# tencent-ailab/pika

Measured on NVIDIA H100. Metric: utterances/sec RNN-T train step (T=1000,U=150,V=6k), higher is better.
Workload: dtype bf16

## Files before the change

pika_b200/csrc/rnnt_loss.cu:

```cuda
#include <cstdlib>

#include "../../include/pika_b200.h"
#include "common.cuh"

namespace pk {
void count_launch();

constexpr float kLog2e = 1.4426950408889634f;
constexpr float kLn2 = 0.6931471805599453f;

template <typename T> struct Vec16;
template <> struct Vec16<__nv_bfloat16> {
    static constexpr int N = 8;
    PK_DEVICE static void unpack(const uint4& q, float (&f)[8]) {
        f[0] = bf16lo(q.x); f[1] = bf16hi(q.x); f[2] = bf16lo(q.y); f[3] = bf16hi(q.y);
        f[4] = bf16lo(q.z); f[5] = bf16hi(q.z); f[6] = bf16lo(q.w); f[7] = bf16hi(q.w);
    }
    PK_DEVICE static uint4 pack(const float (&f)[8]) {
        return make_uint4(pack_bf16x2(f[0], f[1]), pack_bf16x2(f[2], f[3]), pack_bf16x2(f[4], f[5]), pack_bf16x2(f[6], f[7]));
    }
    PK_DEVICE static float vmax(const uint4& q) {
        const __nv_bfloat162 a = __hmax2(*reinterpret_cast<const __nv_bfloat162*>(&q.x), *reinterpret_cast<const __nv_bfloat162*>(&q.y));
        const __nv_bfloat162 b = __hmax2(*reinterpret_cast<const __nv_bfloat162*>(&q.z), *reinterpret_cast<const __nv_bfloat162*>(&q.w));
        const __nv_bfloat162 c = __hmax2(a, b);
        return fmaxf(__low2float(c), __high2float(c));
    }
};
template <> struct Vec16<float> {
    static constexpr int N = 4;
    PK_DEVICE static void unpack(const uint4& q, float (&f)[4]) {
        f[0] = __uint_as_float(q.x); f[1] = __uint_as_float(q.y); f[2] = __uint_as_float(q.z); f[3] = __uint_as_float(q.w);
    }
    PK_DEVICE static uint4 pack(const float (&f)[4]) {
        return make_uint4(__float_as_uint(f[0]), __float_as_uint(f[1]), __float_as_uint(f[2]), __float_as_uint(f[3]));
    }
    PK_DEVICE static float vmax(const uint4& q) {
        return fmaxf(fmaxf(__uint_as_float(q.x), __uint_as_float(q.y)), fmaxf(__uint_as_float(q.z), __uint_as_float(q.w)));
    }
};

PK_DEVICE uint4 ld_stream(const uint4* p) {
    uint4 r;
    asm volatile("ld.global.nc.L1::no_allocate.v4.u32 {%0,%1,%2,%3}, [%4];" : "=r"(r.x), "=r"(r.y), "=r"(r.z), "=r"(r.w) : "l"(p));
    return r;
}
PK_DEVICE uint4 ld_plain(const uint4* p) { return *p; }
PK_DEVICE void st_stream(uint4* p, const uint4& v) {
    asm volatile("st.global.cs.v4.u32 [%0], {%1,%2,%3,%4};" ::"l"(p), "r"(v.x), "r"(v.y), "r"(v.z), "r"(v.w) : "memory");
}

struct RnntDims {
    int B, T, U1, V, ldv;
    int ld_labels;
    int ND;
};
PK_DEVICE size_t skew_index(const RnntDims& d, int b, int t, int u) { return ((size_t)b * d.ND + (t + u)) * d.U1 + u; }

constexpr int ROWSTATS_UNROLL = 4;

template <typename T>
__global__ void __launch_bounds__(256) rnnt_rowstats_kernel(const T* __restrict__ logits, const int* __restrict__ labels,
                                                            const int* __restrict__ frame_lens, const int* __restrict__ label_lens,
                                                            RnntDims d, float* __restrict__ lse_out, float* __restrict__ lpb_skew,
                                                            float* __restrict__ lpl_skew) {
    constexpr int VN = Vec16<T>::N;
    const int lane = threadIdx.x & 31;
    const long long warp_global = (long long)blockIdx.x * (blockDim.x >> 5) + (threadIdx.x >> 5);
    const long long n_warps = (long long)gridDim.x * (blockDim.x >> 5);
    const long long rows = (long long)d.B * d.T * d.U1;
    const int nvec = (d.V + VN - 1) / VN;
    for (long long row = warp_global; row < rows; row += n_warps) {
        const int u = (int)(row % d.U1);
        const long long bt = row / d.U1;
        const int t = (int)(bt % d.T);
        const int b = (int)(bt / d.T);
        const int Tn = frame_lens[b], Un = label_lens[b];
        if (t >= Tn || u > Un) continue;
        const T* rp = logits + row * (long long)d.ldv;
        const uint4* vp = reinterpret_cast<const uint4*>(rp);
        float m = -INFINITY, s = 0.f;
        const int nfull = d.V / VN;
        for (int i0 = lane; i0 < nfull; i0 += 32 * ROWSTATS_UNROLL) {
            uint4 q[ROWSTATS_UNROLL];
#pragma unroll
            for (int k = 0; k < ROWSTATS_UNROLL; ++k) {
                const int i = i0 + k * 32;
                if (i < nfull) q[k] = ld_stream(vp + i);
            }
#pragma unroll
            for (int k = 0; k < ROWSTATS_UNROLL; ++k) {
                const int i = i0 + k * 32;
                if (i < nfull) {
                    const float cm = Vec16<T>::vmax(q[k]) * kLog2e;
                    if (cm > m) { s *= exp2f(m - cm); m = cm; }
                    float f[VN];
                    Vec16<T>::unpack(q[k], f);
#pragma unroll
                    for (int e = 0; e < VN; ++e) s += ex2_approx(fmaf(f[e], kLog2e, -m));
                }
            }
        }
        if (nfull * VN < d.V && lane == 0) {
            for (int v = nfull * VN; v < d.V; ++v) {
                const float x = to_f32<T>(rp[v]) * kLog2e;
                if (x > m) { s *= exp2f(m - x); m = x; }
                s += exp2f(x - m);
            }
        }
        const float mw = warp_max(m);
        s = (m == -INFINITY) ? 0.f : s * exp2f(m - mw);
        s = warp_sum(s);
        if (lane == 0) {
            const float lse = (mw + log2f(s)) * kLn2;
            const float zb = to_f32<T>(rp[0]);
            lse_out[row] = lse;
            const size_t sk = skew_index(d, b, t, u);
            lpb_skew[sk] = zb - lse;
            if (u < Un) {
                const int y = labels[(size_t)b * d.ld_labels + u];
                lpl_skew[sk] = to_f32<T>(rp[y]) - lse;
            }
        }
    }
}

template <typename T>
__global__ void __launch_bounds__(256) rnnt_rowfinish_kernel(const T* __restrict__ logits, const int* __restrict__ labels,
                                                             const int* __restrict__ frame_lens, const int* __restrict__ label_lens,
                                                             RnntDims d, const float2* __restrict__ parts, int n_parts,
                                                             float* __restrict__ lse_out, float* __restrict__ lpb_skew,
                                                             float* __restrict__ lpl_skew) {
    const long long rows = (long long)d.B * d.T * d.U1;
    for (long long row = (long long)blockIdx.x * blockDim.x + threadIdx.x; row < rows; row += (long long)gridDim.x * blockDim.x) {
        const int u = (int)(row % d.U1);
        const long long bt = row / d.U1;
        const int t = (int)(bt % d.T);
        const int b = (int)(bt / d.T);
        const int Tn = frame_lens[b], Un = label_lens[b];
        if (t >= Tn || u > Un) continue;
        float m = -INFINITY;
        for (int i = 0; i < n_parts; ++i) m = fmaxf(m, parts[(size_t)i * rows + row].x);
        float sum = 0.f;
        for (int i = 0; i < n_parts; ++i) {
            const float2 ps = parts[(size_t)i * rows + row];
            sum += ps.y * exp2f(ps.x - m);
        }
        const float lse = (m + log2f(sum)) * kLn2;
        const T* rp = logits + row * (long long)d.ldv;
        lse_out[row] = lse;
        const size_t sk = skew_index(d, b, t, u);
        lpb_skew[sk] = to_f32<T>(rp[0]) - lse;
        if (u < Un) {
            const int y = labels[(size_t)b * d.ld_labels + u];
            lpl_skew[sk] = to_f32<T>(rp[y]) - lse;
        }
    }
}

typedef double lat_t;
#define LAT_NEG_INF (-(double)INFINITY)
PK_DEVICE lat_t lse2(lat_t a, lat_t b) {
    const lat_t mx = fmax(a, b), mn = fmin(a, b);
    if (mx == LAT_NEG_INF) return LAT_NEG_INF;
    return mx + log1p(exp(mn - mx));
}

constexpr int LAT_MAX_G = 512;
constexpr int LAT_MAX_CPT = 4;

__global__ void __launch_bounds__(2 * LAT_MAX_G) rnnt_lattice_kernel(
    const int* __restrict__ frame_lens, const int* __restrict__ label_lens, RnntDims d, int G, int cpt,
    const float* __restrict__ lpb_skew, const float* __restrict__ lpl_skew, lat_t* __restrict__ alpha_skew,
    lat_t* __restrict__ beta_skew, const float* __restrict__ grad_scale, float* __restrict__ costs,
    float* __restrict__ gb_out, float* __restrict__ gl_out) {
    extern __shared__ lat_t sm[];
    const int b = blockIdx.x;
    const int grp = threadIdx.x >= G ? 1 : 0;
    const int j = threadIdx.x - grp * G;
    const int T = frame_lens[b], U = label_lens[b];
    const int W = d.U1 + 2;
    lat_t* buf0 = sm + grp * 2 * W + 1;
    lat_t* buf1 = buf0 + W;
    __shared__ lat_t s_ll;
    const size_t base = (size_t)b * d.ND * d.U1;
    const bool valid = (T > 0 && T <= d.T && U >= 0 && U < d.U1);
    if (valid) {
        for (int i = j - 1; i <= d.U1; i += G) { buf0[i] = LAT_NEG_INF; buf1[i] = LAT_NEG_INF; }
        named_bar_sync(1 + grp, G);
        const int last = T - 1 + U;
        if (grp == 0) {
            lat_t* prev = buf0;
            lat_t* cur = buf1;
            if (j == 0) { cur[0] = 0.0; alpha_skew[base] = 0.0; }
            float nb[LAT_MAX_CPT], nl[LAT_MAX_CPT];
#pragma unroll
            for (int c = 0; c < LAT_MAX_CPT; ++c) {
                const int u = j + c * G;
                nb[c] = (c < cpt && u <= U && last >= 1) ? lpb_skew[base + u] : 0.f;
                nl[c] = (c < cpt && u >= 1 && u <= U && last >= 1) ? lpl_skew[base + u - 1] : 0.f;
            }
            named_bar_sync(1, G);
            for (int dg = 1; dg <= last; ++dg) {
                lat_t* tsw = prev; prev = cur; cur = tsw;
                const int lo = max(0, dg - (T - 1)), hi = min(U, dg);
                float pb[LAT_MAX_CPT], pl[LAT_MAX_CPT];
#pragma unroll
                for (int c = 0; c < LAT_MAX_CPT; ++c) { pb[c] = nb[c]; pl[c] = nl[c]; }
                if (dg < last) {
                    const size_t nbase = base + (size_t)dg * d.U1;
#pragma unroll
                    for (int c = 0; c < LAT_MAX_CPT; ++c) {
                        const int u = j + c * G;
                        if (c < cpt && u <= U) {
                            nb[c] = lpb_skew[nbase + u];
                            nl[c] = (u >= 1) ? lpl_skew[nbase + u - 1] : 0.f;
                        }
                    }
                }
#pragma unroll
                for (int c = 0; c < LAT_MAX_CPT; ++c) {
                    const int u = j + c * G;
                    if (c < cpt && u >= lo && u <= hi) {
                        lat_t a = LAT_NEG_INF, cc = LAT_NEG_INF;
                        if (u <= dg - 1) a = prev[u] + pb[c];
                        if (u >= 1) cc = prev[u - 1] + pl[c];
                        const lat_t v = lse2(a, cc);
                        cur[u] = v;
                        alpha_skew[base + (size_t)dg * d.U1 + u] = v;
                    }
                }
                named_bar_sync(1, G);
            }
        } else {
            lat_t* prev = buf0;
            lat_t* cur = buf1;
            if (j == 0) {
                const lat_t v = lpb_skew[base + (size_t)last * d.U1 + U];
                cur[U] = v;
                beta_skew[base + (size_t)last * d.U1 + U] = v;
            }
            float nb[LAT_MAX_CPT], nl[LAT_MAX_CPT];
#pragma unroll
            for (int c = 0; c < LAT_MAX_CPT; ++c) {
                const int u = j + c * G;
                const bool ok = c < cpt && u <= U && last >= 1;
                nb[c] = ok ? lpb_skew[base + (size_t)(last - 1) * d.U1 + u] : 0.f;
                nl[c] = ok ? lpl_skew[base + (size_t)(last - 1) * d.U1 + u] : 0.f;
            }
            named_bar_sync(2, G);
            for (int dg = last - 1; dg >= 0; --dg) {
                lat_t* tsw = prev; prev = cur; cur = tsw;
                const int lo = max(0, dg - (T - 1)), hi = min(U, dg);
                float pb[LAT_MAX_CPT], pl[LAT_MAX_CPT];
#pragma unroll
                for (int c = 0; c < LAT_MAX_CPT; ++c) { pb[c] = nb[c]; pl[c] = nl[c]; }
                if (dg > 0) {
                    const size_t nbase = base + (size_t)(dg - 1) * d.U1;
#pragma unroll
                    for (int c = 0; c < LAT_MAX_CPT; ++c) {
                        const int u = j + c * G;
                        if (c < cpt && u <= U) { nb[c] = lpb_skew[nbase + u]; nl[c] = lpl_skew[nbase + u]; }
                    }
                }
#pragma unroll
                for (int c = 0; c < LAT_MAX_CPT; ++c) {
                    const int u = j + c * G;
                    if (c < cpt && u >= lo && u <= hi) {
                        const int t = dg - u;
                        lat_t a = LAT_NEG_INF, cc = LAT_NEG_INF;
                        if (t + 1 <= T - 1) a = prev[u] + pb[c];
                        if (u + 1 <= U) cc = prev[u + 1] + pl[c];
                        const lat_t v = lse2(a, cc);
                        cur[u] = v;
                        beta_skew[base + (size_t)dg * d.U1 + u] = v;
                    }
                }
                named_bar_sync(2, G);
            }
            if (j == 0) { s_ll = cur[0]; costs[b] = (float)(-cur[0]); }
        }
    } else if (threadIdx.x == 0) {
        costs[b] = 0.f;
    }
    __syncthreads();
    const float gs = grad_scale ? grad_scale[b] : 1.f;
    const lat_t ll = valid ? s_ll : 0.0;
    const int nodes = d.T * d.U1;
    for (int i = threadIdx.x; i < nodes; i += blockDim.x) {
        const int t = i / d.U1, u = i - t * d.U1;
        float gb = 0.f, gl = 0.f;
        if (valid && t < T && u <= U) {
            const size_t sk = skew_index(d, b, t, u);
            const lat_t a = alpha_skew[sk];
            lat_t bn;
            if (t < T - 1) bn = beta_skew[skew_index(d, b, t + 1, u)];
            else bn = (u == U) ? 0.0 : LAT_NEG_INF;
            gb = (float)(-exp(a + bn + (lat_t)lpb_skew[sk] - ll)) * gs;
            if (u < U) gl = (float)(-exp(a + beta_skew[skew_index(d, b, t, u + 1)] + (lat_t)lpl_skew[sk] - ll)) * gs;
            if (!(gb == gb)) gb = 0.f;
            if (!(gl == gl)) gl = 0.f;
        }
        gb_out[(size_t)b * nodes + i] = gb;
        gl_out[(size_t)b * nodes + i] = gl;
    }
}

constexpr int GRAD_THREADS = 256;
template <typename T> struct GradCfg { static constexpr int MAXG = 32 / Vec16<T>::N; };
template <typename T, int GRAD_RU, int MINB>
__global__ void __launch_bounds__(GRAD_THREADS, MINB) rnnt_grad_kernel(const T* logits, const int* __restrict__ labels,
                                                                    const int* __restrict__ label_lens, RnntDims d,
                                                                    const float* __restrict__ lse_in, const float* __restrict__ gb_in,
                                                                    const float* __restrict__ gl_in, T* dlogits, float* __restrict__ colsum,
                                                                    long long rows_per_cta) {
    constexpr int VN = Vec16<T>::N;
    constexpr int GRAD_MAXG = GradCfg<T>::MAXG;
    extern __shared__ float gsm[];
    float* s_gb = gsm;
    float* s_gl = gsm + rows_per_cta;
    float* s_l2 = gsm + 2 * rows_per_cta;
    int* s_y = reinterpret_cast<int*>(gsm + 3 * rows_per_cta);
    const long long rows = (long long)d.B * d.T * d.U1;
    const long long r0 = (long long)blockIdx.x * rows_per_cta;
    const long long r1 = min(rows, r0 + rows_per_cta);
    const int nvec_ld = d.ldv / VN;
    const int tid = threadIdx.x;
    for (long long row = r0 + tid; row < r1; row += GRAD_THREADS) {
        const int i = (int)(row - r0);
        s_gb[i] = gb_in[row];
        s_gl[i] = gl_in[row];
        s_l2[i] = lse_in[row] * kLog2e;
        const int u = (int)(row % d.U1);
        const int b = (int)(row / ((long long)d.T * d.U1));
        s_y[i] = (u < label_lens[b]) ? labels[(size_t)b * d.ld_labels + u] : -1;
    }
    __syncthreads();
    float cs[GRAD_MAXG][VN];
#pragma unroll
    for (int gq = 0; gq < GRAD_MAXG; ++gq)
#pragma unroll
        for (int e = 0; e < VN; ++e) cs[gq][e] = 0.f;
    for (long long rb = r0; rb < r1; rb += GRAD_RU) {
        uint4 q[GRAD_RU][GRAD_MAXG];
#pragma unroll
        for (int k = 0; k < GRAD_RU; ++k) {
            const long long row = rb + k;
            if (row < r1 && (s_gb[row - r0] != 0.f || s_gl[row - r0] != 0.f)) {
                const uint4* vp = reinterpret_cast<const uint4*>(logits + row * (long long)d.ldv);
#pragma unroll
                for (int gq = 0; gq < GRAD_MAXG; ++gq) {
                    const int i = tid + gq * GRAD_THREADS;
                    if (i < nvec_ld) q[k][gq] = ld_plain(vp + i);
                }
            }
        }
#pragma unroll
        for (int k = 0; k < GRAD_RU; ++k) {
            const long long row = rb + k;
            if (row >= r1) continue;
            const float gb = s_gb[row - r0], gl = s_gl[row - r0];
            uint4* op = reinterpret_cast<uint4*>(dlogits + row * (long long)d.ldv);
            if (gb == 0.f && gl == 0.f) {
#pragma unroll
                for (int gq = 0; gq < GRAD_MAXG; ++gq) {
                    const int i = tid + gq * GRAD_THREADS;
                    if (i < nvec_ld) st_stream(op + i, make_uint4(0, 0, 0, 0));
                }
                continue;
            }
            const int y = s_y[row - r0];
            const float l2 = s_l2[row - r0];
            const float gsum = -(gb + gl);
#pragma unroll
            for (int gq = 0; gq < GRAD_MAXG; ++gq) {
                const int i = tid + gq * GRAD_THREADS;
                if (i < nvec_ld) {
                    float f[VN];
                    Vec16<T>::unpack(q[k][gq], f);
#pragma unroll
                    for (int e = 0; e < VN; ++e) f[e] = ex2_approx(fmaf(f[e], kLog2e, -l2)) * gsum;
                    const int v0 = i * VN;
                    if (v0 == 0) f[0] += gb;
                    if (y >= v0 && y < v0 + VN) {
#pragma unroll
                        for (int e = 0; e < VN; ++e) if (v0 + e == y) f[e] += gl;
                    }
                    if (v0 + VN > d.V) {
#pragma unroll
                        for (int e = 0; e < VN; ++e) if (v0 + e >= d.V) f[e] = 0.f;
                    }
                    const uint4 packed = Vec16<T>::pack(f);
                    st_stream(op + i, packed);
                    if (colsum) {
                        float w[VN];
                        Vec16<T>::unpack(packed, w);
#pragma unroll
                        for (int e = 0; e < VN; ++e) cs[gq][e] += w[e];
                    }
                }
            }
        }
    }
    if (colsum) {
        float* part = colsum + (size_t)blockIdx.x * d.ldv;
#pragma unroll
        for (int gq = 0; gq < GRAD_MAXG; ++gq) {
            const int i = tid + gq * GRAD_THREADS;
            if (i < nvec_ld) {
#pragma unroll
                for (int e = 0; e < VN; ++e) part[i * VN + e] = cs[gq][e];
            }
        }
    }
}

__global__ void __launch_bounds__(256) colsum_partials_kernel(const float* __restrict__ part, int n_part, int ld, float* __restrict__ out) {
    __shared__ float sm[8][33];
    const int tx = threadIdx.x & 31, ty = threadIdx.x >> 5;
    const int c = blockIdx.x * 32 + tx;
    float a = 0.f;
    if (c < ld) {
        const int per = (n_part + 7) / 8;
        const int i0 = ty * per, i1 = min(n_part, i0 + per);
        float a0 = 0.f, a1 = 0.f, a2 = 0.f, a3 = 0.f;
        int i = i0;
        for (; i + 4 <= i1; i += 4) {
            a0 += part[(size_t)(i + 0) * ld + c]; a1 += part[(size_t)(i + 1) * ld + c];
            a2 += part[(size_t)(i + 2) * ld + c]; a3 += part[(size_t)(i + 3) * ld + c];
        }
        for (; i < i1; ++i) a0 += part[(size_t)i * ld + c];
        a = (a0 + a1) + (a2 + a3);
    }
    sm[ty][tx] = a;
    __syncthreads();
    if (ty == 0 && c < ld) {
        float t = sm[0][tx];
#pragma unroll
        for (int k = 1; k < 8; ++k) t += sm[k][tx];
        out[c] = t;
    }
}

}

extern "C" long long pk_rnnt_loss_workspace_bytes(int B, int T, int U1) {
    const long long nd = (long long)T + U1 - 1;
    const long long skew = (long long)B * nd * U1;
    const long long nodes = (long long)B * T * U1;
    return (2 * skew + 3 * nodes) * 4 + 2 * skew * 8 + 256;
}
static void rnnt_grad_grid(long long rows, long long* rpc_out, int* ggrid_out) {
    const int ru = 2;
    const int gcta = pk::num_sms() * 3 * 4;
    long long rpc = (rows + gcta - 1) / gcta;
    rpc = (rpc + ru - 1) / ru * ru;
    if (rpc > 2048) rpc = 2048;
    *rpc_out = rpc; *ggrid_out = (int)((rows + rpc - 1) / rpc);
}
extern "C" long long pk_rnnt_loss_colsum_workspace_bytes(int B, int T, int U1, int ldv) {
    int ggrid; long long rpc;
    rnnt_grad_grid((long long)B * T * U1, &rpc, &ggrid);
    return (long long)ggrid * ldv * 4;
}

static int rnnt_loss_impl(const void* logits, int dtype, const int* labels, const int* frame_lens,
                          const int* label_lens, int B, int T, int U1, int V, int ldv, int ld_labels,
                          const float* grad_scale, float* costs, void* dlogits, float* dlogits_colsum, void* workspace,
                          long long workspace_bytes, const float* row_lse, int n_parts, void* stream_v) {
    using namespace pk;
    cudaStream_t stream = reinterpret_cast<cudaStream_t>(stream_v);
    PK_CHECK_ARG(dtype == PK_F32 || dtype == PK_BF16, "bad dtype");
    PK_CHECK_ARG(B > 0 && T > 0 && U1 > 0 && V > 1, "bad dims");
    const int vn = dtype == PK_F32 ? 4 : 8;
    PK_CHECK_ARG(ldv >= V && ldv % vn == 0, "ldv must be >= V and a multiple of 16 bytes");
    PK_CHECK_ARG((reinterpret_cast<uintptr_t>(logits) & 15) == 0, "logits not 16B aligned");
    PK_CHECK_ARG(dlogits == nullptr || (reinterpret_cast<uintptr_t>(dlogits) & 15) == 0, "dlogits not 16B aligned");
    PK_CHECK_ARG(workspace_bytes >= pk_rnnt_loss_workspace_bytes(B, T, U1), "workspace too small");
    RnntDims d{B, T, U1, V, ldv, ld_labels, T + U1 - 1};
    const size_t skew = (size_t)B * d.ND * U1, nodes = (size_t)B * T * U1;
    double* wsd = reinterpret_cast<double*>(workspace);
    double* alpha = wsd; double* beta = alpha + skew;
    float* lpb = reinterpret_cast<float*>(beta + skew); float* lpl = lpb + skew;
    float* lse = lpl + skew; float* gb = lse + nodes; float* gl = gb + nodes;

    const long long rows = (long long)nodes;
    const int warps_per_cta = 8;
    long long want = (rows + warps_per_cta - 1) / warps_per_cta;
    const long long cap = (long long)num_sms() * 8 * 4;
    const int grid = (int)(want < cap ? want : cap);
    if (row_lse != nullptr) {
        PK_CHECK_ARG(n_parts >= 1, "n_parts must be >= 1");
        const int fgrid = (int)((rows + 255) / 256 < (long long)num_sms() * 8 ? (rows + 255) / 256 : (long long)num_sms() * 8);
        if (dtype == PK_BF16)
            rnnt_rowfinish_kernel<__nv_bfloat16><<<fgrid, 256, 0, stream>>>(reinterpret_cast<const __nv_bfloat16*>(logits), labels, frame_lens,
                                                                           label_lens, d, reinterpret_cast<const float2*>(row_lse), n_parts,
                                                                           lse, lpb, lpl);
        else
            rnnt_rowfinish_kernel<float><<<fgrid, 256, 0, stream>>>(reinterpret_cast<const float*>(logits), labels, frame_lens, label_lens, d,
                                                                   reinterpret_cast<const float2*>(row_lse), n_parts, lse, lpb, lpl);
    } else if (dtype == PK_BF16)
        rnnt_rowstats_kernel<__nv_bfloat16><<<grid, 256, 0, stream>>>(reinterpret_cast<const __nv_bfloat16*>(logits), labels,
                                                                     frame_lens, label_lens, d, lse, lpb, lpl);
    else
        rnnt_rowstats_kernel<float><<<grid, 256, 0, stream>>>(reinterpret_cast<const float*>(logits), labels, frame_lens,
                                                              label_lens, d, lse, lpb, lpl);
    PK_CHECK_LAUNCH(); count_launch();
    const int lat_smem = 2 * 2 * (U1 + 2) * 8;
    int G = ((U1 + 31) / 32) * 32;
    if (G > LAT_MAX_G) G = LAT_MAX_G;
    const int cpt = (U1 + G - 1) / G;
    PK_CHECK_ARG(cpt <= LAT_MAX_CPT, "U too large for the lattice kernel (U+1 <= 2048)");
    static bool configured = false;
    if (!configured) {
        PK_CHECK_CUDA(cudaFuncSetAttribute(rnnt_lattice_kernel, cudaFuncAttributeMaxDynamicSharedMemorySize,
                                           2 * 2 * (LAT_MAX_G * LAT_MAX_CPT + 2) * (int)sizeof(lat_t)));
        configured = true;
    }
    rnnt_lattice_kernel<<<B, 2 * G, lat_smem, stream>>>(frame_lens, label_lens, d, G, cpt, lpb, lpl, alpha, beta, grad_scale,
                                                     costs, gb, gl);
    PK_CHECK_LAUNCH(); count_launch();
    if (dlogits != nullptr) {
        PK_CHECK_ARG(ldv <= 8192, "V too large for the gradient kernel (V <= 8192)");
        int ggrid; long long rpc;
        rnnt_grad_grid(rows, &rpc, &ggrid);
        float* cs_part = nullptr;
        if (dlogits_colsum) {
            const long long base_bytes = pk_rnnt_loss_workspace_bytes(B, T, U1);
            PK_CHECK_ARG(workspace_bytes >= base_bytes + (long long)ggrid * ldv * 4,
                         "workspace too small for the column sums (add pk_rnnt_loss_colsum_workspace_bytes)");
            cs_part = reinterpret_cast<float*>(reinterpret_cast<unsigned char*>(workspace) + base_bytes);
        }
        const size_t gsmem = (size_t)rpc * 16;
#define PK_GRAD_LAUNCH(TT, RU, MB)                                                                                         \
        rnnt_grad_kernel<TT, RU, MB><<<ggrid, GRAD_THREADS, gsmem, stream>>>(reinterpret_cast<const TT*>(logits), labels, label_lens, d, lse, \
                                                                            gb, gl, reinterpret_cast<TT*>(dlogits), cs_part, rpc)
        if (dtype == PK_BF16) PK_GRAD_LAUNCH(__nv_bfloat16, 2, 3);
        else PK_GRAD_LAUNCH(float, 2, 2);
#undef PK_GRAD_LAUNCH
        PK_CHECK_LAUNCH(); count_launch();
        if (dlogits_colsum) {
            colsum_partials_kernel<<<(ldv + 31) / 32, 256, 0, stream>>>(cs_part, ggrid, ldv, dlogits_colsum);
            PK_CHECK_LAUNCH(); count_launch();
        }
    }
    return 0;
}

extern "C" int pk_rnnt_loss_fwd_bwd(const void* logits, int dtype, const int* labels, const int* frame_lens,
                                    const int* label_lens, int B, int T, int U1, int V, int ldv, int ld_labels,
                                    const float* grad_scale, float* costs, void* dlogits, float* dlogits_colsum, void* workspace,
                                    long long workspace_bytes, void* stream) {
    return rnnt_loss_impl(logits, dtype, labels, frame_lens, label_lens, B, T, U1, V, ldv, ld_labels, grad_scale, costs, dlogits,
                          dlogits_colsum, workspace, workspace_bytes, nullptr, 0, stream);
}

extern "C" int pk_rnnt_loss_fwd_bwd_lse(const void* logits, int dtype, const int* labels, const int* frame_lens,
                                        const int* label_lens, int B, int T, int U1, int V, int ldv, int ld_labels,
                                        const float* grad_scale, float* costs, void* dlogits, float* dlogits_colsum, void* workspace,
                                        long long workspace_bytes, const float* row_lse, int n_parts, void* stream) {
    PK_CHECK_ARG(row_lse != nullptr, "row_lse is null");
    return rnnt_loss_impl(logits, dtype, labels, frame_lens, label_lens, B, T, U1, V, ldv, ld_labels, grad_scale, costs, dlogits,
                          dlogits_colsum, workspace, workspace_bytes, row_lse, n_parts, stream);
}
```

Baseline: 197.2.

## Double-buffer row loads in RNN-T grad kernel and specialize vector groups by V

Splits the gradient kernel loop into load and compute lambdas and adds a register double-buffered prefetch path, so the next rows' logits are loaded while the current rows' gradients are computed. Makes the per-thread vector group count a template parameter and picks 3 groups with 3-row unroll for bf16 when ldv fits, otherwise 4 groups, with min blocks lowered to 2. The aim is to hide global memory latency in this bandwidth-bound kernel, at the cost of doubled register buffers and possibly lower occupancy. The prefetch reads past r1 are guarded by the row bounds check.

```diff
diff --git a/pika_b200/csrc/rnnt_loss.cu b/pika_b200/csrc/rnnt_loss.cu
--- a/pika_b200/csrc/rnnt_loss.cu
+++ b/pika_b200/csrc/rnnt_loss.cu
@@ -1,4 +1,3 @@
-#include <cstdlib>
 
 #include "../../include/pika_b200.h"
 #include "common.cuh"
@@ -306,15 +305,13 @@
 }
 
 constexpr int GRAD_THREADS = 256;
-template <typename T> struct GradCfg { static constexpr int MAXG = 32 / Vec16<T>::N; };
-template <typename T, int GRAD_RU, int MINB>
+template <typename T, int GRAD_RU, int MINB, bool PREFETCH, int GRAD_MAXG>
 __global__ void __launch_bounds__(GRAD_THREADS, MINB) rnnt_grad_kernel(const T* logits, const int* __restrict__ labels,
                                                                     const int* __restrict__ label_lens, RnntDims d,
                                                                     const float* __restrict__ lse_in, const float* __restrict__ gb_in,
                                                                     const float* __restrict__ gl_in, T* dlogits, float* __restrict__ colsum,
                                                                     long long rows_per_cta) {
     constexpr int VN = Vec16<T>::N;
-    constexpr int GRAD_MAXG = GradCfg<T>::MAXG;
     extern __shared__ float gsm[];
     float* s_gb = gsm;
     float* s_gl = gsm + rows_per_cta;
@@ -340,8 +337,7 @@
     for (int gq = 0; gq < GRAD_MAXG; ++gq)
 #pragma unroll
         for (int e = 0; e < VN; ++e) cs[gq][e] = 0.f;
-    for (long long rb = r0; rb < r1; rb += GRAD_RU) {
-        uint4 q[GRAD_RU][GRAD_MAXG];
+    auto load_rows = [&](long long rb, uint4 (&q)[GRAD_RU][GRAD_MAXG]) {
 #pragma unroll
         for (int k = 0; k < GRAD_RU; ++k) {
             const long long row = rb + k;
@@ -354,6 +350,8 @@
                 }
             }
         }
+    };
+    auto grad_rows = [&](long long rb, const uint4 (&q)[GRAD_RU][GRAD_MAXG]) {
 #pragma unroll
         for (int k = 0; k < GRAD_RU; ++k) {
             const long long row = rb + k;
@@ -399,6 +397,22 @@
                     }
                 }
             }
+        }
+    };
+    if constexpr (PREFETCH) {
+        uint4 qa[GRAD_RU][GRAD_MAXG], qb[GRAD_RU][GRAD_MAXG];
+        load_rows(r0, qa);
+        for (long long rb = r0; rb < r1; rb += 2 * GRAD_RU) {
+            load_rows(rb + GRAD_RU, qb);
+            grad_rows(rb, qa);
+            load_rows(rb + 2 * GRAD_RU, qa);
+            grad_rows(rb + GRAD_RU, qb);
+        }
+    } else {
+        for (long long rb = r0; rb < r1; rb += GRAD_RU) {
+            uint4 q[GRAD_RU][GRAD_MAXG];
+            load_rows(rb, q);
+            grad_rows(rb, q);
         }
     }
     if (colsum) {
@@ -531,11 +545,12 @@
             cs_part = reinterpret_cast<float*>(reinterpret_cast<unsigned char*>(workspace) + base_bytes);
         }
         const size_t gsmem = (size_t)rpc * 16;
-#define PK_GRAD_LAUNCH(TT, RU, MB)                                                                                         \
-        rnnt_grad_kernel<TT, RU, MB><<<ggrid, GRAD_THREADS, gsmem, stream>>>(reinterpret_cast<const TT*>(logits), labels, label_lens, d, lse, \
-                                                                            gb, gl, reinterpret_cast<TT*>(dlogits), cs_part, rpc)
-        if (dtype == PK_BF16) PK_GRAD_LAUNCH(__nv_bfloat16, 2, 3);
-        else PK_GRAD_LAUNCH(float, 2, 2);
+#define PK_GRAD_LAUNCH(TT, RU, MB, PF, G)                                                                                  \
+        rnnt_grad_kernel<TT, RU, MB, PF, G><<<ggrid, GRAD_THREADS, gsmem, stream>>>(reinterpret_cast<const TT*>(logits), labels, label_lens, d, \
+                                                                                   lse, gb, gl, reinterpret_cast<TT*>(dlogits), cs_part, rpc)
+        if (dtype == PK_BF16 && ldv <= 3 * GRAD_THREADS * 8) PK_GRAD_LAUNCH(__nv_bfloat16, 3, 2, true, 3);
+        else if (dtype == PK_BF16) PK_GRAD_LAUNCH(__nv_bfloat16, 2, 2, true, 4);
+        else PK_GRAD_LAUNCH(float, 2, 2, false, 8);
 #undef PK_GRAD_LAUNCH
         PK_CHECK_LAUNCH(); count_launch();
         if (dlogits_colsum) {
```

Result: no change. 197.5 (median of 6 runs) (+0.1%).
